# hidasib/GRU4Rec

Measured on NVIDIA H100. Metric: mini-batches/sec, higher is better.
Workload: dtype f32

## Files before the change

### gru4rec_b200/csrc/g4r_fast.cuh

```cuda
#pragma once

constexpr int FK_THREADS = 512;
constexpr int FK_NW = FK_THREADS / 32;
constexpr int FK_G = 48;
constexpr int FK_CT = 32;
constexpr int FK_Q = FK_CT / FK_NW;
constexpr int FK_B = 32;
static_assert(FK_THREADS / 16 == FK_B, "statistics mapping: 16 threads per lane");
constexpr int FK_LDS = 132;


__device__ __forceinline__ void red_release_add(unsigned int* p, unsigned int v) {
  asm volatile("red.release.gpu.global.add.u32 [%0], %1;" :: "l"(p), "r"(v) : "memory");
}
__device__ __forceinline__ unsigned int atom_acqrel_add(unsigned int* p, unsigned int v) {
  unsigned int old;
  asm volatile("atom.acq_rel.gpu.global.add.u32 %0, [%1], %2;" : "=r"(old) : "l"(p), "r"(v) : "memory");
  return old;
}
__device__ __forceinline__ void wait_ge(const unsigned int* p, unsigned int target) {
  while (ld_acquire_u32(p) < target) { }
}
__device__ __forceinline__ uint32_t smem_u32(const void* p) { return (uint32_t)__cvta_generic_to_shared(p); }
__device__ __forceinline__ void mbar_init(uint64_t* bar, unsigned int count) {
// ... 42 lines not shown
  const int tid = threadIdx.x;
  if (s >= n_steps) return;
  const int M = md.wM[s];
  const int* cbeg = md.pCbeg + (size_t)s * (md.NCH + 1);
  const bool hc = chunk < md.NCH;
  const int cb = hc ? cbeg[chunk] : 0, ce = hc ? cbeg[chunk + 1] : 0;
  if (tid < FK_CT) {
    int it = 0, pos = 0;
    if (cb + tid < ce) { it = md.pItem[(size_t)s * md.NP + cb + tid]; pos = md.pPos[(size_t)s * md.NP + cb + tid]; }
    sm.sIt[buf][tid] = it; sm.sPos[buf][tid] = pos;
  }
  if (tid >= 32 && tid < 32 + FK_B) {
    const int b = tid - 32;
    sm.sTc[buf][b] = b < M ? md.pTcol[(size_t)s * md.B + b] : -1;
    sm.sYit[buf][b] = b < M ? md.wY[(size_t)s * md.B + b] : 0;
  }
  if (tid == 64) { sm.sCb[buf][0] = cb; sm.sCb[buf][1] = ce; }
}

template <class SM>
__device__ __forceinline__ void fk_prefetch_rows(const ModelDev& md, SM& sm, int s, int n_steps, int buf, bool pw) {
  if (s >= n_steps) return;
  const int tid = threadIdx.x;
  const int M = md.wM[s];
  const int cb = sm.sCb[buf][0], ce = sm.sCb[buf][1];
  const int nj = ce - cb;
  const bool ada = md.adapt == G4R_ADAPT_ADAGRAD, mom = md.mom > 0.f;
  const unsigned int rowb = (unsigned int)md.ldL * 4u;
  uint64_t* bar = reinterpret_cast<uint64_t*>(&sm.mbar);
  const int ntab = 1 + (ada ? 1 : 0) + (mom ? 1 : 0);
  const int ncopy = nj * ntab + (pw ? M : 0);
  if (tid == 0) {
    const unsigned int total = rowb * (unsigned int)ncopy;
    asm volatile("fence.proxy.async.global;" ::: "memory");
    if (total > 0) mbar_expect_tx(bar, total);
    else asm volatile("mbarrier.arrive.shared::cta.b64 _, [%0];" :: "r"(smem_u32(bar)) : "memory");
  }
  if ((tid & 31) == 0) {
    for (int i = tid >> 5; i < ncopy; i += FK_NW) {
      if (i < nj * ntab) {
        const int j = i / ntab, t = i % ntab;
        const size_t off = (size_t)sm.sIt[buf][j] * md.ldL;
        if (t == 0) tma_row(sm.sS + j * FK_LDS, md.Wy + off, rowb, bar);
        else if (t == 1 && ada) tma_row(sm.sAcc + j * FK_LDS, md.Wy_acc + off, rowb, bar);
        else tma_row(sm.sVel + j * FK_LDS, md.Wy_vel + off, rowb, bar);
      } else {
        const int b = i - nj * ntab;
        tma_row(sm.sTW + b * FK_LDS, md.Wy + (size_t)sm.sYit[buf][b] * md.ldL, rowb, bar);
      }
    }
  }
  if (false) {
  } else if (tid >= 64 && tid < 64 + FK_CT) {
    const int j = tid - 64;
    if (j < nj) {
      const int it = sm.sIt[buf][j];
      float bz = md.By[it];
      sm.sByP[j] = bz;
      if (md.logq > 0.f) bz -= (sm.sPos[buf][j] < M) ? md.logP0t[it] : md.logP0s[it];
      sm.sBias[j] = bz;
      sm.sByA[j] = ada ? md.By_acc[it] : 0.f;
      sm.sByV[j] = mom ? md.By_vel[it] : 0.f;
    }
  } else if (tid >= 96 && tid < 96 + FK_B) {
    const int b = tid - 96;
    if (pw && b < M) {
      const int it = sm.sYit[buf][b];
      float bz = md.By[it];
      if (md.logq > 0.f) bz -= md.logP0t[it];
      sm.sTB[b] = bz;
    }
// ... 556 lines not shown
        if (m == 0) { sc = sm.sD + k0 + j; ss = FK_LDS; } else { sc = (m == 1 ? sm.gDr : sm.gDz) + j; ss = FR_U; }
        o = jm * FK_LDS + q * 4;
      } else {
        vec = sm.sD + q * 4; sc = sm.gHr + k0 + j; ss = FK_LDS;
        o = j * FK_LDS + q * 4;
      }
      float4 g = make_float4(0.f, 0.f, 0.f, 0.f);
#pragma unroll 4
      for (int b = 0; b < M; b++) {
        const float4 a = ld4(vec + b * FK_LDS);
        const float d = sc[b * ss];
        g.x = fmaf(a.x, d, g.x); g.y = fmaf(a.y, d, g.y); g.z = fmaf(a.z, d, g.z); g.w = fmaf(a.w, d, g.w);
      }
      if (k0 + j < L) {
        float* P = colt ? sm.rC[0] : sm.rR[0];
        float* A = colt ? sm.rC[1] : sm.rR[1];
        float* V = colt ? sm.rC[2] : sm.rR[2];
        if (q * 4 + 0 < L) fr_upd(md, ada, mom, g.x, P[o + 0], A[o + 0], V[o + 0]);
        if (q * 4 + 1 < L) fr_upd(md, ada, mom, g.y, P[o + 1], A[o + 1], V[o + 1]);
        if (q * 4 + 2 < L) fr_upd(md, ada, mom, g.z, P[o + 2], A[o + 2], V[o + 2]);
        if (q * 4 + 3 < L) fr_upd(md, ada, mom, g.w, P[o + 3], A[o + 3], V[o + 3]);
      }
    } else {
      const int i = t - ncol - nrow, m = i / FR_U, j = i % FR_U;
      if (k0 + j < L) {
        float g = 0.f;
        for (int b = 0; b < M; b++) g = g + (m == 0 ? sm.sD[b * FK_LDS + k0 + j] : (m == 1 ? sm.gDr : sm.gDz)[b * FR_U + j]);
        fr_upd(md, ada, mom, g, sm.rB[0][i], sm.rB[1][i], sm.rB[2][i]);
      }
    }
  }
}
template <class SM>
__device__ __forceinline__ void fk_stage_y(const ModelDev& md, SM& sm, int M, float* hnext) {
  const LayerDev& ly = md.layer[0];
  const int ldL = ly.ldL, kw = ldL / 4, n1 = FK_B * kw, total = hnext ? 2 * n1 : n1;
  for (int i0 = 0; i0 < total; i0 += 4 * FK_THREADS) {
    float4 v[4];
#pragma unroll
    for (int u = 0; u < 4; u++) {
      const int i = i0 + u * FK_THREADS + (int)threadIdx.x;
      v[u] = make_float4(0.f, 0.f, 0.f, 0.f);
      if (i < n1) { const int rr = i / kw; if (rr < M) v[u] = ld4(ly.y + (size_t)rr * ldL + (i % kw) * 4); }
      else if (i < total) { const int sl = sm.gIdx[(i - n1) / kw]; if (sl >= 0) v[u] = ld4(ly.H + (size_t)sl * ldL + ((i - n1) % kw) * 4); }
    }
#pragma unroll
    for (int u = 0; u < 4; u++) {
      const int i = i0 + u * FK_THREADS + (int)threadIdx.x;
      if (i < n1) st4(sm.sY + (i / kw) * FK_LDS + (i % kw) * 4, v[u]);
      else if (i < total) st4(hnext + ((i - n1) / kw) * FK_LDS + ((i - n1) % kw) * 4, v[u]);
    }
  }
}

#include "g4r_fastc.cuh"

template <bool CL>
__global__ void __launch_bounds__(FK_THREADS, 1) k_fast_t(int slot, int n_steps, FastSync* fs, unsigned long long* tstamp) {
  using SM = typename std::conditional<CL, FastSmemC, FastSmemR>::type;
  extern __shared__ __align__(128) unsigned char fk_raw[];
  SM& sm = *reinterpret_cast<SM*>(fk_raw);
  const ModelDev& md = MD;
  const LayerDev& ly = md.layer[0];
  const int cta = blockIdx.x, ncta = gridDim.x;
  const int tid = threadIdx.x, lane = tid & 31, warp = tid >> 5;
  const int chunk = cta;
  const bool has_chunk = chunk < md.NCH;
  const int G = CL ? (int)cl_size() : md.ldL / 4;
  const bool gru = cta < G;
  const bool pw = loss_pairwise(md.loss);
  const bool ada = md.adapt == G4R_ADAPT_ADAGRAD, mom = md.mom > 0.f;
  const int ldL = md.ldL, B = md.B;
  const int kw = ldL / 4;
  uint64_t* bar = reinterpret_cast<uint64_t*>(&sm.mbar);
  unsigned int bar_epoch = 0, gepoch = 0, stats_target = 0;
  const int in_ctas = min(B, ncta - G);
#ifdef G4R_CF_FINE
#define FK_FTS(s_) ((tstamp && cta == 0 && (s_) < 500 && n_steps >= 1000) ? tstamp + (size_t)((s_) + 500) * 16 : nullptr)
#define FK_STAMP_OK(s_) ((s_) < 500)
#else
#define FK_FTS(s_) ((unsigned long long*)nullptr)
#define FK_STAMP_OK(s_) true
#endif
#define FK_STAMP(k) do { if (tstamp && cta == 0 && tid == 0 && FK_STAMP_OK(s)) { unsigned long long t_; asm volatile("mov.u64 %0, %%globaltimer;" : "=l"(t_)); tstamp[(size_t)s * 16 + (k)] = t_; } } while (0)
  if (tid == 0) { mbar_init(bar, 1); asm volatile("fence.mbarrier_init.release.cluster;" ::: "memory"); }
  fk_load_idx(md, sm, 0, n_steps, chunk, 0);
  __syncthreads();
  fk_prefetch_rows(md, sm, 0, n_steps, 0, pw);
  ClusterCtx cc = {0, 1, 0, 0};
  if constexpr (CL) {
    if (gru) {
      cc = cf_init(md, sm);
      cf_load_resident(md, sm, cc);
      if (n_steps > 0) {
        fk_stage_lanes(md, sm, 0, md.wM[0]);
        cf_f1(md, sm, cc, 0, false, nullptr, 0u, nullptr);
        cf_f2(md, sm, cc, 0, nullptr);
        __syncthreads();
        if (tid == 0) red_release_add(&fs->h_ready, 1u);
      }
    }
  } else {
    if (gru) {
      fr_load_resident(md, sm, 4 * cta);
      if (n_steps > 0) {
        fk_stage_lanes(md, sm, 0, md.wM[0]);
        stage_rows4(sm.gH[0], FK_LDS, FK_B, kw, [&](int rr) -> const float* { const int sl = sm.gIdx[rr]; return sl >= 0 ? ly.H + (size_t)sl * ldL : nullptr; });
        fr_f1(md, sm, 0, 4 * cta, sm.gH[0], nullptr, 0u);
        fk_group_barrier(fs, gepoch, G);
        fr_f2(md, sm, 0, 4 * cta, sm.gH[0]);
        __syncthreads();
        if (tid == 0) red_release_add(&fs->h_ready, 1u);
      }
    }
  }
  for (int s = 0; s < n_steps; s++) {
    const int buf = s & 1;
    const int M = md.wM[s];
    const int sti = md.wSti[s];
    const int N = M + (sti >= 0 ? md.S : 0);
    FK_STAMP(0);
    fk_load_idx(md, sm, s + 1, n_steps, chunk, buf ^ 1);
    const bool gru_next = !CL && gru && s + 1 < n_steps;
    if (gru_next && tid < FK_B) {
      const int M1 = md.wM[s + 1];
      sm.gIdx[tid] = tid < M1 ? md.wSlot[(size_t)(s + 1) * B + tid] : -1;
      sm.gIdx[FK_B + tid] = tid < M1 ? md.wX[(size_t)(s + 1) * B + tid] : 0;
      sm.gIdx[2 * FK_B + tid] = tid < M1 ? md.wF[(size_t)(s + 1) * B + tid] : 0;
    }
    if (tid == 0) wait_ge(&fs->h_ready, (unsigned int)(s + 1) * (unsigned int)G);
    __syncthreads();
    if constexpr (CL) stage_rows4(sm.sY, FK_LDS, FK_B, kw, [&](int rr) -> const float* { return rr < M ? ly.y + (size_t)rr * ldL : nullptr; });
    else fk_stage_y(md, sm, M, gru_next ? sm.gH[(s + 1) & 1] : nullptr);
    mbar_wait(bar, (unsigned int)(s & 1));
    __syncthreads();
    FK_STAMP(1);
    const int cb = sm.sCb[buf][0], ce = sm.sCb[buf][1];
    const int nj = ce - cb;
    if (pw) {
      for (int b = warp; b < FK_B; b += FK_NW) {
        if (b < M) {
          float a = 0.f;
          if (lane < kw) {
            const float4 y = ld4(sm.sY + b * FK_LDS + lane * 4), w = ld4(sm.sTW + b * FK_LDS + lane * 4);
            a = fmaf(w.x, y.x, a); a = fmaf(w.y, y.y, a); a = fmaf(w.z, y.z, a); a = fmaf(w.w, y.w, a);
          }
          a = warp_sum(a);
          if (lane == 0) sm.sT[b] = act_fwd(md.fact, a + sm.sTB[b]);
        }
      }
    }
    {
      float accq[FK_Q];
#pragma unroll
      for (int q = 0; q < FK_Q; q++) accq[q] = 0.f;
      const float* yr = sm.sY + lane * FK_LDS;
      for (int c4 = 0; c4 < kw; c4++) {
        const float4 y = ld4(yr + c4 * 4);
#pragma unroll
        for (int q = 0; q < FK_Q; q++) {
          if (warp + FK_NW * q < nj) {
            const float4 w = ld4(sm.sS + (warp + FK_NW * q) * FK_LDS + c4 * 4);
            accq[q] = fmaf(y.x, w.x, accq[q]); accq[q] = fmaf(y.y, w.y, accq[q]); accq[q] = fmaf(y.z, w.z, accq[q]); accq[q] = fmaf(y.w, w.w, accq[q]);
          }
        }
      }
// ... 88 lines not shown
        const float m = mg;
        float* rs = md.RS + (size_t)b * G4R_NSTAT;
        float loss = 0.f, r0 = m, r1 = Z, r2 = 0.f, r3 = 0.f, r4 = 0.f, r5 = tt;
        if (md.loss == G4R_LOSS_XE) { const float pt = __fdiv_rn(expf(T - m), Z); loss = -logf(pt + G4R_EPS_LOG); r2 = pt; r5 = T; }
        else if (md.loss == G4R_LOSS_XE_LOGIT) { loss = logf(Z) - (T - m); r5 = T; }
        else if (md.loss == G4R_LOSS_BPR_MAX) { r2 = __fdiv_rn(A, Z); r3 = __fdiv_rn(Q, Z); r4 = __fdiv_rn(D, Z); loss = -logf(r2 + G4R_EPS_LOG) + md.bpreg * r3; }
        else if (md.loss == G4R_LOSS_TOP1_MAX) { r2 = __fdiv_rn(A, Z); r4 = __fdiv_rn(D, Z); loss = r2; }
        else if (md.loss == G4R_LOSS_BPR) { loss = A; r4 = D; }
        else { const float c = sigmoidf_(tt * tt); loss = (float)M * (__fdiv_rn(A, (float)N) - __fdiv_rn(c, (float)(M + md.S_cfg))); r4 = D; }
        st4(rs, make_float4(r0, r1, r2, r3));
        st4(rs + 4, make_float4(r4, r5, loss, 0.f));
        red_release_add(&fs->stats, 1u);
      }
    }
    stats_target += (unsigned int)M;
    if (tid == 0) wait_ge(&fs->stats, stats_target);
    __syncthreads();
    FK_STAMP(2);
    if (tid < M * 2) st4(sm.sRS + tid * 4, ld4(md.RS + tid * 4));
    __syncthreads();
    if (chunk == 0 && tid == 0) {
      float c = 0.f;
      for (int b = 0; b < M; b++) c += sm.sRS[b * 8 + 6];
      c = __fdiv_rn(c, (float)md.B);
      md.cost[s] = c;
      if (c != c) atomicExch(md.nanflag, 1);
    }
    FK_STAMP(11);
    for (int i = tid; i < FK_CT * FK_B; i += FK_THREADS) {
      const int jj = i / FK_B, b = i % FK_B;
      sm.sG[i] = (jj < nj && b < M) ? loss_grad_elem(md, sm.sRS + (size_t)b * 8, sm.sO[i], sm.sTc[buf][b] == cb + jj, M, N) : 0.f;
    }
    __syncthreads();
    for (int jj = warp; jj < nj; jj += FK_THREADS / 32) {
      float a = (lane < M) ? sm.sG[jj * FK_B + lane] : 0.f;
      a = warp_sum(a);
      if (lane == 0) sm.sDby[jj] = a;
    }
    FK_STAMP(12);
    float* part = md.part + (size_t)(has_chunk ? chunk : 0) * md.B * ldL;
    if (has_chunk) {
      for (int t = tid; t < nj * kw; t += FK_THREADS) {
        const int jj = t / kw, q4 = t % kw;
        float4 d = make_float4(0.f, 0.f, 0.f, 0.f);
        for (int bb = 0; bb < M; bb++) {
          const float4 y = ld4(sm.sY + bb * FK_LDS + q4 * 4);
          const float g = sm.sG[jj * FK_B + bb];
          d.x = fmaf(g, y.x, d.x); d.y = fmaf(g, y.y, d.y); d.z = fmaf(g, y.z, d.z); d.w = fmaf(g, y.w, d.w);
        }
        st4(sm.sD + jj * FK_LDS + q4 * 4, d);
      }
      for (int t = tid; t < M * kw; t += FK_THREADS) {
        const int bb = t / kw, q4 = t % kw;
        float4 a = make_float4(0.f, 0.f, 0.f, 0.f);
        for (int jj = 0; jj < nj; jj++) {
          const float g = sm.sG[jj * FK_B + bb];
          const float4 w = ld4(sm.sS + jj * FK_LDS + q4 * 4);
          a.x = fmaf(g, w.x, a.x); a.y = fmaf(g, w.y, a.y); a.z = fmaf(g, w.z, a.z); a.w = fmaf(g, w.w, a.w);
        }
        st4(part + (size_t)bb * ldL + q4 * 4, a);
      }
    }
    __syncthreads();
    FK_STAMP(13);
    for (int j = warp; j < nj; j += FK_THREADS / 32) {
      const int item = sm.sIt[buf][j];
      if (j > 0 && sm.sIt[buf][j - 1] == item) continue;
      int je = j + 1;
      while (je < nj && sm.sIt[buf][je] == item) je++;
      if (lane < kw) {
        const float4 p0 = ld4(sm.sS + j * FK_LDS + lane * 4);
        float4 a0 = make_float4(0.f, 0.f, 0.f, 0.f), v0 = a0, al = a0, vl = a0;
        if (ada) a0 = ld4(sm.sAcc + j * FK_LDS + lane * 4);
        if (mom) v0 = ld4(sm.sVel + j * FK_LDS + lane * 4);
        float4 ps = p0;
        for (int k = j; k < je; k++) {
          const float4 g = ld4(sm.sD + k * FK_LDS + lane * 4);
          float4 gs = g;
          if (ada) {
            al.x = a0.x + g.x * g.x; al.y = a0.y + g.y * g.y; al.z = a0.z + g.z * g.z; al.w = a0.w + g.w * g.w;
            gs.x = __fdiv_rn(g.x, sqrtf(al.x + G4R_EPS_ADA)); gs.y = __fdiv_rn(g.y, sqrtf(al.y + G4R_EPS_ADA));
            gs.z = __fdiv_rn(g.z, sqrtf(al.z + G4R_EPS_ADA)); gs.w = __fdiv_rn(g.w, sqrtf(al.w + G4R_EPS_ADA));
          }
          float4 d;
          if (md.lmbd > 0.f) { d.x = md.lr * (gs.x + md.lmbd * p0.x); d.y = md.lr * (gs.y + md.lmbd * p0.y); d.z = md.lr * (gs.z + md.lmbd * p0.z); d.w = md.lr * (gs.w + md.lmbd * p0.w); }
          else { d.x = md.lr * gs.x; d.y = md.lr * gs.y; d.z = md.lr * gs.z; d.w = md.lr * gs.w; }
          if (mom) {
            vl.x = md.mom * v0.x - d.x; vl.y = md.mom * v0.y - d.y; vl.z = md.mom * v0.z - d.z; vl.w = md.mom * v0.w - d.w;
            ps.x += vl.x; ps.y += vl.y; ps.z += vl.z; ps.w += vl.w;
          } else { ps.x -= d.x; ps.y -= d.y; ps.z -= d.z; ps.w -= d.w; }
        }
        const size_t off = (size_t)item * ldL + lane * 4;
        st4(md.Wy + off, ps);
        if (ada) st4(md.Wy_acc + off, al);
        if (mom) st4(md.Wy_vel + off, vl);
      }
      if (lane == 0) {
        const float p0 = sm.sByP[j];
        float a0 = sm.sByA[j], v0 = sm.sByV[j], al = 0.f, vl = 0.f, ps = p0;
        for (int k = j; k < je; k++) {
          const float g = sm.sDby[k];
          float gs = g;
          if (ada) { al = a0 + g * g; gs = __fdiv_rn(g, sqrtf(al + G4R_EPS_ADA)); }
          const float d = md.lmbd > 0.f ? md.lr * (gs + md.lmbd * p0) : md.lr * gs;
          if (mom) { vl = md.mom * v0 - d; ps += vl; } else ps -= d;
        }
        md.By[item] = ps;
        if (ada) md.By_acc[item] = al;
        if (mom) md.By_vel[item] = vl;
      }
    }
    if (has_chunk && nj == 0) for (int i = tid; i < M * ldL; i += FK_THREADS) part[i] = 0.f;
    __syncthreads();
    FK_STAMP(14);
    bar_epoch += 1;
    if (tid == 0) { red_release_add(&fs->bar, 1u); wait_ge(&fs->bar, bar_epoch * (unsigned int)ncta); }
    __syncthreads();
    FK_STAMP(3);
    fk_b1<CL>(md, sm, s, cta, ncta);
    __syncthreads();
    if (tid == 0) red_release_add(&fs->b1_done, 1u);
    FK_STAMP(15);
    fk_prefetch_rows(md, sm, s + 1, n_steps, buf ^ 1, pw);
    FK_STAMP(4);
    if constexpr (CL) {
      if (gru) {
        if (s + 1 < n_steps) fk_stage_lanes(md, sm, s + 1, md.wM[s + 1]);
        cf_backward(md, sm, cc, fs, s, ncta, s + 1 < n_steps, (tstamp && cta == 0 && FK_STAMP_OK(s)) ? tstamp + (size_t)s * 16 : nullptr, FK_FTS(s));
        FK_STAMP(6);
        if (s + 1 < n_steps) {
          cf_f1(md, sm, cc, s + 1, true, &fs->in_done, (unsigned int)(s + 1) * (unsigned int)in_ctas, FK_FTS(s));
          FK_STAMP(7);
          cf_f2(md, sm, cc, s + 1, FK_FTS(s));
          __syncthreads();
          if (tid == 0) red_release_add(&fs->h_ready, 1u);
        } else {
          cl_wait();
        }
        FK_STAMP(8);
      }
    } else if (gru) {
      const int k0 = 4 * cta;
      const float* sHo = sm.gH[s & 1];
      if (tid == 0) wait_ge(&fs->b1_done, (unsigned int)(s + 1) * (unsigned int)ncta);
      __syncthreads();
      fr_b2(md, sm, s, k0, sHo);
      __syncthreads();
      if (tid == 0) red_release_add(&fs->dvec_done, 1u);
      FK_STAMP(5);
      fr_dense(md, sm, s, k0, sHo);
      FK_STAMP(6);
      if (s + 1 < n_steps) {
        fr_f1(md, sm, s + 1, k0, sm.gH[(s + 1) & 1], &fs->in_done, (unsigned int)(s + 1) * (unsigned int)in_ctas);
        fk_group_barrier(fs, gepoch, G);
        FK_STAMP(7);
        fr_f2(md, sm, s + 1, k0, sm.gH[(s + 1) & 1]);
        __syncthreads();
        if (tid == 0) red_release_add(&fs->h_ready, 1u);
      }
      FK_STAMP(8);
    }
    if (!gru && cta < G + in_ctas) {
      const unsigned int* ctr = CL ? &fs->grp : &fs->dvec_done;
      const unsigned int tgt = (unsigned int)(s + 1) * (unsigned int)G;
      if (in_ctas == B && ly.ld3 / 4 <= FK_THREADS) fk_sparse_in_one(md, sm, s, cta - G, ctr, tgt);
      else {
        if (tid == 0) wait_ge(ctr, tgt);
        __syncthreads();
        for (int b = cta - G; b < B; b += in_ctas) { fk_sparse_in(md, sm, s, b); __syncthreads(); }
      }
      __syncthreads();
      if (tid == 0) red_release_add(&fs->in_done, 1u);
    }
  }
  if constexpr (CL) { if (gru) cf_store_resident(md, sm, cc); }
  else { if (gru) fr_store_resident(md, sm, 4 * cta); }
#undef FK_STAMP
}
```

### gru4rec_b200/csrc/g4r_kernels.cuh

```cuda
#pragma once
#include <cuda_runtime.h>
#include <stdint.h>
#include "../../include/g4r.h"

#define G4R_EPS_ADA 1e-6f
#define G4R_EPS_LOG 1e-24f
#define G4R_NSTAT 8

struct ActSpec { int kind; float p1, p2; };
constexpr int MG_CAP = 256;
struct MgDev {
  int R, rank;
  int *gItem, *gPos, *gM, *gX;
  int *mEnt, *mItem, *mCbeg;
  int *mTot;
  int *xEnt, *xItem, *xTot;
  float *DSYall, *DBYall, *INall;
  float* gradFlat; size_t gradCount;
};

struct MgTensor { float *p, *acc, *vel; size_t goff; int count; };
struct TsBuf {
  unsigned char *A1, *A2, *A3, *A4, *A5, *A6, *A7, *A8;
  unsigned char *W1, *W2, *W3, *W4, *B3, *B4, *B5, *B8a, *B8b;
// ... 25 lines not shown
  return t;
}

constexpr int MGS_MAXR = 8;
constexpr int MGS_FLAG_STRIDE = 32;
constexpr int MGS_GRU_CTAS = 48;
enum { MGF_ROWS = 0, MGF_APPLIED = MGS_MAXR, MGF_IN = 2 * MGS_MAXR, MGF_INAPPLIED = 3 * MGS_MAXR, MGF_DENSE = 4 * MGS_MAXR,
       MGF_COUNT = 4 * MGS_MAXR + MGS_MAXR * MGS_GRU_CTAS };
struct ShardDev {
  int R, rank, rows_local, ldW;
  int NA, DSL;
  float* W[MGS_MAXR];
  float* Wx[MGS_MAXR];
  float* inbox[MGS_MAXR];
  float* inboxIn[MGS_MAXR];
  float* denseIn[MGS_MAXR];
  float* mgInLL[MGS_MAXR];
  unsigned int* flags[MGS_MAXR];
  float *W_acc, *W_vel, *Wx_acc, *Wx_vel;
  float* mgIn;
  const int *aEnt, *aItem, *aCbeg;
  const int *xEnt, *xItem, *xTot;
  const int *gX, *gM;
  int* abort;
};
struct FastSync {
  unsigned int bar;      unsigned int p0[31];
  unsigned int stats;    unsigned int p1[31];
  unsigned int h_ready;  unsigned int p2[31];
  unsigned int b1_done;  unsigned int p3[31];
  unsigned int grp;      unsigned int p4[31];
  unsigned int in_done;  unsigned int p5[31];
  unsigned int dvec_done; unsigned int p6[31];
};
struct GridBar { unsigned int count; unsigned int gen; unsigned int pad[30]; };

struct LayerDev {
  int L, ldL, ld2, ld3;
  int in_dim, ld_in;
  float *Wx, *Wx_acc, *Wx_vel;
  float *Wh, *Wh_acc, *Wh_vel;
  float *Wrz, *Wrz_acc, *Wrz_vel;
  float *Bh, *Bh_acc, *Bh_vel;
  float *Wx_g, *Wh_g, *Wrz_g, *Bh_g;
  float *H;
  float *Hold, *r, *z, *ah, *ht, *y;
  float *dvec;
  float *dy;
  float *Hr;
  const float* in;
};

struct ModelDev {
  int n_items, n_layers, B, Bld, S, mode;
  int L, ldL;
  int in0_dim, ld_in0;
  int NP;
  int NCH;
  int loss; ActSpec fact, hact;
  float p_drop_h, p_drop_e, lr, mom, lmbd, bpreg, logq, alpha;
  int adapt; int nn_top1;
  float ap1, ap1c, ap2, ap2c;
  float grad_cap, smoothing;
  const float* gscale;
  float* gnorm2;
  float* stat2;
// ... 1238 lines not shown
```

### gru4rec_b200/csrc/g4r_lib.cu

```cuda
#include <cuda_runtime.h>
#include <algorithm>
#include <cmath>
#include <cstdio>
#include <cstring>
#include <map>
#include <mutex>
#include <string>
#include <vector>
#include "g4r_kernels.cuh"
#include "g4r_misc.cuh"

#define G4R_VERSION 100

static thread_local std::string g_create_error;
struct g4r_handle;
static void eval_release(g4r_handle* h);
static void mg_release(g4r_handle* h);
static void shard_release(g4r_handle* h);
static bool shard_eligible(const g4r_config& c, int n_sm);
static int shard_create(g4r_handle* h);
static bool tc_eligible(const g4r_config& c);
struct TensorInfo;
static int shard_set_tensor(g4r_handle* h, const TensorInfo& t, const float* host);
static int shard_get_tensor(g4r_handle* h, const TensorInfo& t, float* host);
// ... 674 lines not shown
  if (h->two_pass) h->md.export_only = 1;
  if (slot_upload(h->slot, h->md, h->stream) != cudaSuccess) return bail(G4R_ERR_CUDA, "constant upload failed");
  const int B = cfg->batch_size, CAP = h->CAP;
  bool ok = true;
  ok &= cudaMallocHost(&h->hX, (size_t)CAP * B * sizeof(int)) == cudaSuccess;
  ok &= cudaMallocHost(&h->hY, (size_t)CAP * B * sizeof(int)) == cudaSuccess;
  ok &= cudaMallocHost(&h->hSlot, (size_t)CAP * B * sizeof(int)) == cudaSuccess;
  ok &= cudaMallocHost(&h->hF, (size_t)CAP * B) == cudaSuccess;
  ok &= cudaMallocHost(&h->hM, (size_t)CAP * sizeof(int)) == cudaSuccess;
  ok &= cudaMallocHost(&h->hSti, (size_t)CAP * sizeof(int)) == cudaSuccess;
  ok &= cudaMallocHost(&h->hG, (size_t)CAP * sizeof(uint32_t)) == cudaSuccess;
  ok &= cudaMallocHost(&h->hCost, (size_t)CAP * sizeof(float)) == cudaSuccess;
  if (!ok) return bail(G4R_ERR_CUDA, "pinned host allocation failed");
  h->pk_smem = std::max(std::max(score_smem_bytes(h->md.Bld), lossgrad_smem_bytes(h->md.Bld, h->md.ldL)), (size_t)2 * GK * (GB + 1) * sizeof(float));
  if (raise_smem_limit((const void*)k_score, score_smem_bytes(h->md.Bld)) != cudaSuccess ||
      raise_smem_limit((const void*)k_lossgrad, lossgrad_smem_bytes(h->md.Bld, h->md.ldL)) != cudaSuccess ||
      raise_smem_limit((const void*)k_plan, (size_t)h->npow2 * 8 + 1024) != cudaSuccess ||
      raise_smem_limit((const void*)k_persistent, h->pk_smem) != cudaSuccess)
    return bail(G4R_ERR_INVALID, "this shape needs more shared memory per block than the device offers (batch_size / layer width / n_sample too large for the step scratch)");
  {
    int per_sm = 0;
    cudaOccupancyMaxActiveBlocksPerMultiprocessor(&per_sm, k_persistent, PK_THREADS, h->pk_smem);
    int coop = 0; cudaDeviceGetAttribute(&coop, cudaDevAttrCooperativeLaunch, cfg->device);
    h->pk_blocks = (per_sm >= 1 && coop) ? h->n_sm : 0;
  }
  {
    const ModelDev& m = h->md;
    raise_smem_limit((const void*)k_fast_t<false>, sizeof(FastSmemR));
    int per_sm = 0;
    cudaOccupancyMaxActiveBlocksPerMultiprocessor(&per_sm, k_fast_t<false>, FK_THREADS, sizeof(FastSmemR));
    const bool plain_opt = m.adapt <= G4R_ADAPT_ADAGRAD && !h->phase_only;
    h->fast_ok = plain_opt && h->pk_blocks > 0 && per_sm >= 1 && m.mode == 0 && m.n_layers == 1 && m.ldL <= 128 && m.B <= FK_B && h->n_sm >= FK_G + 1 && m.NCH <= 160 &&
                 2 * m.L <= FK_W1 * FK_G && m.L <= FK_W2 * FK_G &&
                 (m.adapt == G4R_ADAPT_ADAGRAD ? m.Wy_acc != nullptr : true);
    h->fastc_ok = plain_opt && cfg->step_mode == 3 && h->fastc_grid >= FC_CLUSTER * 2 && m.mode == 0 && m.n_layers == 1 && m.ldL <= 128 && m.B <= FK_B &&
                  m.NCH <= h->fastc_grid && (m.adapt == G4R_ADAPT_ADAGRAD ? m.Wy_acc != nullptr : true);
    cudaMallocHost(&h->hFlags, 4 * sizeof(int));
  }
  if (h->tc_ok) {
    if (ts_opt_in(h) != G4R_OK) return bail(G4R_ERR_CUDA, "k_ts_gemm: shared memory / cluster opt-in failed");
    h->fast_ok = false; h->fastc_ok = false;
  }
  if (cfg->step_mode == 1 && h->pk_blocks == 0) return bail(G4R_ERR_INVALID, "persistent mode unavailable (cooperative launch / shared memory)");
  if (h->md.shardR > 0) {
    const int src = shard_create(h);
    if (src) return bail(src, h->err);
    h->fast_ok = false; h->fastc_ok = false;
  }
  if (cudaStreamSynchronize(h->stream) != cudaSuccess) return bail(G4R_ERR_CUDA, "init sync failed");
  *out = h;
  return G4R_OK;
}

extern "C" void* g4r_stream(g4r_handle* h) { return h ? (void*)h->stream : nullptr; }
extern "C" int64_t g4r_kernel_launches(const g4r_handle* h) { return h ? h->launches : 0; }

static TensorInfo* find_tensor(g4r_handle* h, const char* name) {
  auto it = h->tensors.find(name ? name : "");
  return it == h->tensors.end() ? nullptr : &it->second;
}
extern "C" int g4r_tensor_shape(g4r_handle* h, const char* name, int64_t* rows, int64_t* cols) {
  if (!h) return G4R_ERR_INVALID;
  TensorInfo* t = find_tensor(h, name);
  if (!t) FAIL(G4R_ERR_INVALID, std::string("unknown tensor ") + (name ? name : "(null)"));
  if (rows) *rows = t->rows;
  if (cols) *cols = t->cols;
// ... 555 lines not shown
```

Before: 28450.

## Offload GRU CTAs' output-row updates to partner CTAs in the non-cluster fast kernel

In the non-cluster persistent kernel, GRU-owning CTAs no longer compute dS·y or apply the output-embedding optimizer updates. They write their loss gradients to global memory, and a dedicated partner CTA fetches them and performs the row updates. That lets the GRU CTAs move straight on to the barrier and the recurrent backward/forward work on the critical path. A new rows_done counter orders the next step's TMA row prefetch after all row updates finish, and next-step H staging moves into the GRU branch. The change needs extra CTAs (a new eligibility check), adds a global round-trip of gradients and extra syncs, and moves the async-proxy fence onto each issuing warp.

```diff
diff --git a/gru4rec_b200/csrc/g4r_fast.cuh b/gru4rec_b200/csrc/g4r_fast.cuh
--- a/gru4rec_b200/csrc/g4r_fast.cuh
+++ b/gru4rec_b200/csrc/g4r_fast.cuh
@@ -98,11 +98,11 @@
   const int ncopy = nj * ntab + (pw ? M : 0);
   if (tid == 0) {
     const unsigned int total = rowb * (unsigned int)ncopy;
-    asm volatile("fence.proxy.async.global;" ::: "memory");
     if (total > 0) mbar_expect_tx(bar, total);
     else asm volatile("mbarrier.arrive.shared::cta.b64 _, [%0];" :: "r"(smem_u32(bar)) : "memory");
   }
   if ((tid & 31) == 0) {
+    asm volatile("fence.proxy.async.global;" ::: "memory");
     for (int i = tid >> 5; i < ncopy; i += FK_NW) {
       if (i < nj * ntab) {
         const int j = i / ntab, t = i % ntab;
@@ -725,25 +725,130 @@
   }
 }
 template <class SM>
-__device__ __forceinline__ void fk_stage_y(const ModelDev& md, SM& sm, int M, float* hnext) {
-  const LayerDev& ly = md.layer[0];
-  const int ldL = ly.ldL, kw = ldL / 4, n1 = FK_B * kw, total = hnext ? 2 * n1 : n1;
-  for (int i0 = 0; i0 < total; i0 += 4 * FK_THREADS) {
-    float4 v[4];
-#pragma unroll
-    for (int u = 0; u < 4; u++) {
-      const int i = i0 + u * FK_THREADS + (int)threadIdx.x;
-      v[u] = make_float4(0.f, 0.f, 0.f, 0.f);
-      if (i < n1) { const int rr = i / kw; if (rr < M) v[u] = ld4(ly.y + (size_t)rr * ldL + (i % kw) * 4); }
-      else if (i < total) { const int sl = sm.gIdx[(i - n1) / kw]; if (sl >= 0) v[u] = ld4(ly.H + (size_t)sl * ldL + ((i - n1) % kw) * 4); }
-    }
-#pragma unroll
-    for (int u = 0; u < 4; u++) {
-      const int i = i0 + u * FK_THREADS + (int)threadIdx.x;
-      if (i < n1) st4(sm.sY + (i / kw) * FK_LDS + (i % kw) * 4, v[u]);
-      else if (i < total) st4(hnext + ((i - n1) / kw) * FK_LDS + ((i - n1) % kw) * 4, v[u]);
-    }
-  }
+__device__ __forceinline__ void fk_part(SM& sm, float* part, int M, int nj, int ldL) {
+  const int kw = ldL / 4;
+  for (int t = threadIdx.x; t < M * kw; t += FK_THREADS) {
+    const int bb = t / kw, q4 = t % kw;
+    float4 a = make_float4(0.f, 0.f, 0.f, 0.f);
+    for (int jj = 0; jj < nj; jj++) {
+      const float g = sm.sG[jj * FK_B + bb];
+      const float4 w = ld4(sm.sS + jj * FK_LDS + q4 * 4);
+      a.x = fmaf(g, w.x, a.x); a.y = fmaf(g, w.y, a.y); a.z = fmaf(g, w.z, a.z); a.w = fmaf(g, w.w, a.w);
+    }
+    st4(part + (size_t)bb * ldL + q4 * 4, a);
+  }
+}
+template <class SM>
+__device__ __forceinline__ void fk_dsy(SM& sm, int M, int nj, int kw) {
+  for (int t = threadIdx.x; t < nj * kw; t += FK_THREADS) {
+    const int jj = t / kw, q4 = t % kw;
+    float4 d = make_float4(0.f, 0.f, 0.f, 0.f);
+    for (int bb = 0; bb < M; bb++) {
+      const float4 y = ld4(sm.sY + bb * FK_LDS + q4 * 4);
+      const float g = sm.sG[jj * FK_B + bb];
+      d.x = fmaf(g, y.x, d.x); d.y = fmaf(g, y.y, d.y); d.z = fmaf(g, y.z, d.z); d.w = fmaf(g, y.w, d.w);
+    }
+    st4(sm.sD + jj * FK_LDS + q4 * 4, d);
+  }
+}
+template <class SM>
+__device__ __forceinline__ void fk_update_rows(const ModelDev& md, SM& sm, int buf, int nj, int kw) {
+  const int lane = threadIdx.x & 31, warp = threadIdx.x >> 5, ldL = md.ldL;
+  const bool ada = md.adapt == G4R_ADAPT_ADAGRAD, mom = md.mom > 0.f;
+  for (int j = warp; j < nj; j += FK_NW) {
+    const int item = sm.sIt[buf][j];
+    if (j > 0 && sm.sIt[buf][j - 1] == item) continue;
+    int je = j + 1;
+    while (je < nj && sm.sIt[buf][je] == item) je++;
+    if (lane < kw) {
+      const float4 p0 = ld4(sm.sS + j * FK_LDS + lane * 4);
+      float4 a0 = make_float4(0.f, 0.f, 0.f, 0.f), v0 = a0, al = a0, vl = a0;
+      if (ada) a0 = ld4(sm.sAcc + j * FK_LDS + lane * 4);
+      if (mom) v0 = ld4(sm.sVel + j * FK_LDS + lane * 4);
+      float4 ps = p0;
+      for (int k = j; k < je; k++) {
+        const float4 g = ld4(sm.sD + k * FK_LDS + lane * 4);
+        float4 gs = g;
+        if (ada) {
+          al.x = a0.x + g.x * g.x; al.y = a0.y + g.y * g.y; al.z = a0.z + g.z * g.z; al.w = a0.w + g.w * g.w;
+          gs.x = __fdiv_rn(g.x, sqrtf(al.x + G4R_EPS_ADA)); gs.y = __fdiv_rn(g.y, sqrtf(al.y + G4R_EPS_ADA));
+          gs.z = __fdiv_rn(g.z, sqrtf(al.z + G4R_EPS_ADA)); gs.w = __fdiv_rn(g.w, sqrtf(al.w + G4R_EPS_ADA));
+        }
+        float4 d;
+        if (md.lmbd > 0.f) { d.x = md.lr * (gs.x + md.lmbd * p0.x); d.y = md.lr * (gs.y + md.lmbd * p0.y); d.z = md.lr * (gs.z + md.lmbd * p0.z); d.w = md.lr * (gs.w + md.lmbd * p0.w); }
+        else { d.x = md.lr * gs.x; d.y = md.lr * gs.y; d.z = md.lr * gs.z; d.w = md.lr * gs.w; }
+        if (mom) {
+          vl.x = md.mom * v0.x - d.x; vl.y = md.mom * v0.y - d.y; vl.z = md.mom * v0.z - d.z; vl.w = md.mom * v0.w - d.w;
+          ps.x += vl.x; ps.y += vl.y; ps.z += vl.z; ps.w += vl.w;
+        } else { ps.x -= d.x; ps.y -= d.y; ps.z -= d.z; ps.w -= d.w; }
+      }
+      const size_t off = (size_t)item * ldL + lane * 4;
+      st4(md.Wy + off, ps);
+      if (ada) st4(md.Wy_acc + off, al);
+      if (mom) st4(md.Wy_vel + off, vl);
+    }
+    if (lane == 0) {
+      const float p0 = sm.sByP[j];
+      float a0 = sm.sByA[j], v0 = sm.sByV[j], al = 0.f, vl = 0.f, ps = p0;
+      for (int k = j; k < je; k++) {
+        const float g = sm.sDby[k];
+        float gs = g;
+        if (ada) { al = a0 + g * g; gs = __fdiv_rn(g, sqrtf(al + G4R_EPS_ADA)); }
+        const float d = md.lmbd > 0.f ? md.lr * (gs + md.lmbd * p0) : md.lr * gs;
+        if (mom) { vl = md.mom * v0 - d; ps += vl; } else ps -= d;
+      }
+      md.By[item] = ps;
+      if (ada) md.By_acc[item] = al;
+      if (mom) md.By_vel[item] = vl;
+    }
+  }
+}
+template <class SM>
+__device__ __forceinline__ void fk_dby(SM& sm, int M, int nj) {
+  const int lane = threadIdx.x & 31, warp = threadIdx.x >> 5;
+  for (int jj = warp; jj < nj; jj += FK_NW) {
+    float a = (lane < M) ? sm.sG[jj * FK_B + lane] : 0.f;
+    a = warp_sum(a);
+    if (lane == 0) sm.sDby[jj] = a;
+  }
+}
+struct FkPartner { int nj, it; float g[2]; };
+__device__ __forceinline__ FkPartner fk_partner_fetch(const ModelDev& md, int s, int g, int M) {
+  const int tid = threadIdx.x;
+  const int* cbeg = md.pCbeg + (size_t)s * (md.NCH + 1);
+  const int cb = g < md.NCH ? cbeg[g] : 0;
+  FkPartner r;
+  r.nj = g < md.NCH ? cbeg[g + 1] - cb : 0;
+  r.it = (tid < r.nj) ? md.pItem[(size_t)s * md.NP + cb + tid] : 0;
+#pragma unroll
+  for (int u = 0; u < 2; u++) {
+    const int i = u * FK_THREADS + tid, jj = i / FK_B, b = i % FK_B;
+    r.g[u] = (jj < r.nj && b < M) ? md.O[(size_t)(cb + jj) * md.Bld + b] : 0.f;
+  }
+  return r;
+}
+template <class SM>
+__device__ int fk_partner_stage(const ModelDev& md, SM& sm, const FkPartner& r, int buf, int M, int kw) {
+  static_assert(FK_CT * FK_B == 2 * FK_THREADS, "fk_partner_fetch: two dL/do entries per thread");
+  const int tid = threadIdx.x, lane = tid & 31, warp = tid >> 5, nj = r.nj;
+  const bool ada = md.adapt == G4R_ADAPT_ADAGRAD, mom = md.mom > 0.f;
+  __syncthreads();
+  if (tid < FK_CT) sm.sIt[buf][tid] = r.it;
+  sm.sG[tid] = r.g[0]; sm.sG[FK_THREADS + tid] = r.g[1];
+  __syncthreads();
+  for (int j = warp; j < nj; j += FK_NW) {
+    const int it = sm.sIt[buf][j];
+    const size_t off = (size_t)it * md.ldL + lane * 4;
+    if (lane < kw) {
+      st4(sm.sS + j * FK_LDS + lane * 4, ld4(md.Wy + off));
+      if (ada) st4(sm.sAcc + j * FK_LDS + lane * 4, ld4(md.Wy_acc + off));
+      if (mom) st4(sm.sVel + j * FK_LDS + lane * 4, ld4(md.Wy_vel + off));
+    }
+    if (lane == 0) { sm.sByP[j] = md.By[it]; sm.sByA[j] = ada ? md.By_acc[it] : 0.f; sm.sByV[j] = mom ? md.By_vel[it] : 0.f; }
+  }
+  asm volatile("fence.proxy.async.shared::cta;" ::: "memory");
+  fk_dby(sm, M, nj);
+  return nj;
 }
 
 #include "g4r_fastc.cuh"
@@ -762,12 +867,12 @@
   const int G = CL ? (int)cl_size() : md.ldL / 4;
   const bool gru = cta < G;
   const bool pw = loss_pairwise(md.loss);
-  const bool ada = md.adapt == G4R_ADAPT_ADAGRAD, mom = md.mom > 0.f;
   const int ldL = md.ldL, B = md.B;
   const int kw = ldL / 4;
   uint64_t* bar = reinterpret_cast<uint64_t*>(&sm.mbar);
   unsigned int bar_epoch = 0, gepoch = 0, stats_target = 0;
   const int in_ctas = min(B, ncta - G);
+  const int partner_of = (!CL && cta >= G + in_ctas && cta < 2 * G + in_ctas) ? cta - G - in_ctas : -1;
 #ifdef G4R_CF_FINE
 #define FK_FTS(s_) ((tstamp && cta == 0 && (s_) < 500 && n_steps >= 1000) ? tstamp + (size_t)((s_) + 500) * 16 : nullptr)
 #define FK_STAMP_OK(s_) ((s_) < 500)
@@ -823,8 +928,7 @@
     }
     if (tid == 0) wait_ge(&fs->h_ready, (unsigned int)(s + 1) * (unsigned int)G);
     __syncthreads();
-    if constexpr (CL) stage_rows4(sm.sY, FK_LDS, FK_B, kw, [&](int rr) -> const float* { return rr < M ? ly.y + (size_t)rr * ldL : nullptr; });
-    else fk_stage_y(md, sm, M, gru_next ? sm.gH[(s + 1) & 1] : nullptr);
+    stage_rows4(sm.sY, FK_LDS, FK_B, kw, [&](int rr) -> const float* { return rr < M ? ly.y + (size_t)rr * ldL : nullptr; });
     mbar_wait(bar, (unsigned int)(s & 1));
     __syncthreads();
     FK_STAMP(1);
@@ -979,98 +1083,34 @@
       sm.sG[i] = (jj < nj && b < M) ? loss_grad_elem(md, sm.sRS + (size_t)b * 8, sm.sO[i], sm.sTc[buf][b] == cb + jj, M, N) : 0.f;
     }
     __syncthreads();
-    for (int jj = warp; jj < nj; jj += FK_THREADS / 32) {
-      float a = (lane < M) ? sm.sG[jj * FK_B + lane] : 0.f;
-      a = warp_sum(a);
-      if (lane == 0) sm.sDby[jj] = a;
+    if (!CL && gru) {
+      for (int i = tid; i < nj * FK_B; i += FK_THREADS) {
+        const int jj = i / FK_B, b = i % FK_B;
+        if (b < M) md.O[(size_t)(cb + jj) * md.Bld + b] = sm.sG[i];
+      }
+    } else {
+      fk_dby(sm, M, nj);
     }
     FK_STAMP(12);
     float* part = md.part + (size_t)(has_chunk ? chunk : 0) * md.B * ldL;
-    if (has_chunk) {
-      for (int t = tid; t < nj * kw; t += FK_THREADS) {
-        const int jj = t / kw, q4 = t % kw;
-        float4 d = make_float4(0.f, 0.f, 0.f, 0.f);
-        for (int bb = 0; bb < M; bb++) {
-          const float4 y = ld4(sm.sY + bb * FK_LDS + q4 * 4);
-          const float g = sm.sG[jj * FK_B + bb];
-          d.x = fmaf(g, y.x, d.x); d.y = fmaf(g, y.y, d.y); d.z = fmaf(g, y.z, d.z); d.w = fmaf(g, y.w, d.w);
-        }
-        st4(sm.sD + jj * FK_LDS + q4 * 4, d);
-      }
-      for (int t = tid; t < M * kw; t += FK_THREADS) {
-        const int bb = t / kw, q4 = t % kw;
-        float4 a = make_float4(0.f, 0.f, 0.f, 0.f);
-        for (int jj = 0; jj < nj; jj++) {
-          const float g = sm.sG[jj * FK_B + bb];
-          const float4 w = ld4(sm.sS + jj * FK_LDS + q4 * 4);
-          a.x = fmaf(g, w.x, a.x); a.y = fmaf(g, w.y, a.y); a.z = fmaf(g, w.z, a.z); a.w = fmaf(g, w.w, a.w);
-        }
-        st4(part + (size_t)bb * ldL + q4 * 4, a);
-      }
-    }
-    __syncthreads();
-    FK_STAMP(13);
-    for (int j = warp; j < nj; j += FK_THREADS / 32) {
-      const int item = sm.sIt[buf][j];
-      if (j > 0 && sm.sIt[buf][j - 1] == item) continue;
-      int je = j + 1;
-      while (je < nj && sm.sIt[buf][je] == item) je++;
-      if (lane < kw) {
-        const float4 p0 = ld4(sm.sS + j * FK_LDS + lane * 4);
-        float4 a0 = make_float4(0.f, 0.f, 0.f, 0.f), v0 = a0, al = a0, vl = a0;
-        if (ada) a0 = ld4(sm.sAcc + j * FK_LDS + lane * 4);
-        if (mom) v0 = ld4(sm.sVel + j * FK_LDS + lane * 4);
-        float4 ps = p0;
-        for (int k = j; k < je; k++) {
-          const float4 g = ld4(sm.sD + k * FK_LDS + lane * 4);
-          float4 gs = g;
-          if (ada) {
-            al.x = a0.x + g.x * g.x; al.y = a0.y + g.y * g.y; al.z = a0.z + g.z * g.z; al.w = a0.w + g.w * g.w;
-            gs.x = __fdiv_rn(g.x, sqrtf(al.x + G4R_EPS_ADA)); gs.y = __fdiv_rn(g.y, sqrtf(al.y + G4R_EPS_ADA));
-            gs.z = __fdiv_rn(g.z, sqrtf(al.z + G4R_EPS_ADA)); gs.w = __fdiv_rn(g.w, sqrtf(al.w + G4R_EPS_ADA));
-          }
-          float4 d;
-          if (md.lmbd > 0.f) { d.x = md.lr * (gs.x + md.lmbd * p0.x); d.y = md.lr * (gs.y + md.lmbd * p0.y); d.z = md.lr * (gs.z + md.lmbd * p0.z); d.w = md.lr * (gs.w + md.lmbd * p0.w); }
-          else { d.x = md.lr * gs.x; d.y = md.lr * gs.y; d.z = md.lr * gs.z; d.w = md.lr * gs.w; }
-          if (mom) {
-            vl.x = md.mom * v0.x - d.x; vl.y = md.mom * v0.y - d.y; vl.z = md.mom * v0.z - d.z; vl.w = md.mom * v0.w - d.w;
-            ps.x += vl.x; ps.y += vl.y; ps.z += vl.z; ps.w += vl.w;
-          } else { ps.x -= d.x; ps.y -= d.y; ps.z -= d.z; ps.w -= d.w; }
-        }
-        const size_t off = (size_t)item * ldL + lane * 4;
-        st4(md.Wy + off, ps);
-        if (ada) st4(md.Wy_acc + off, al);
-        if (mom) st4(md.Wy_vel + off, vl);
-      }
-      if (lane == 0) {
-        const float p0 = sm.sByP[j];
-        float a0 = sm.sByA[j], v0 = sm.sByV[j], al = 0.f, vl = 0.f, ps = p0;
-        for (int k = j; k < je; k++) {
-          const float g = sm.sDby[k];
-          float gs = g;
-          if (ada) { al = a0 + g * g; gs = __fdiv_rn(g, sqrtf(al + G4R_EPS_ADA)); }
-          const float d = md.lmbd > 0.f ? md.lr * (gs + md.lmbd * p0) : md.lr * gs;
-          if (mom) { vl = md.mom * v0 - d; ps += vl; } else ps -= d;
-        }
-        md.By[item] = ps;
-        if (ada) md.By_acc[item] = al;
-        if (mom) md.By_vel[item] = vl;
-      }
-    }
-    if (has_chunk && nj == 0) for (int i = tid; i < M * ldL; i += FK_THREADS) part[i] = 0.f;
-    __syncthreads();
-    FK_STAMP(14);
-    bar_epoch += 1;
-    if (tid == 0) { red_release_add(&fs->bar, 1u); wait_ge(&fs->bar, bar_epoch * (unsigned int)ncta); }
-    __syncthreads();
-    FK_STAMP(3);
-    fk_b1<CL>(md, sm, s, cta, ncta);
-    __syncthreads();
-    if (tid == 0) red_release_add(&fs->b1_done, 1u);
-    FK_STAMP(15);
-    fk_prefetch_rows(md, sm, s + 1, n_steps, buf ^ 1, pw);
-    FK_STAMP(4);
     if constexpr (CL) {
+      if (has_chunk) { fk_dsy(sm, M, nj, kw); fk_part(sm, part, M, nj, ldL); }
+      __syncthreads();
+      FK_STAMP(13);
+      fk_update_rows(md, sm, buf, nj, kw);
+      if (has_chunk && nj == 0) for (int i = tid; i < M * ldL; i += FK_THREADS) part[i] = 0.f;
+      __syncthreads();
+      FK_STAMP(14);
+      bar_epoch += 1;
+      if (tid == 0) { red_release_add(&fs->bar, 1u); wait_ge(&fs->bar, bar_epoch * (unsigned int)ncta); }
+      __syncthreads();
+      FK_STAMP(3);
+      fk_b1<CL>(md, sm, s, cta, ncta);
+      __syncthreads();
+      if (tid == 0) red_release_add(&fs->b1_done, 1u);
+      FK_STAMP(15);
+      fk_prefetch_rows(md, sm, s + 1, n_steps, buf ^ 1, pw);
+      FK_STAMP(4);
       if (gru) {
         if (s + 1 < n_steps) fk_stage_lanes(md, sm, s + 1, md.wM[s + 1]);
         cf_backward(md, sm, cc, fs, s, ncta, s + 1 < n_steps, (tstamp && cta == 0 && FK_STAMP_OK(s)) ? tstamp + (size_t)s * 16 : nullptr, FK_FTS(s));
@@ -1086,38 +1126,87 @@
         }
         FK_STAMP(8);
       }
-    } else if (gru) {
-      const int k0 = 4 * cta;
-      const float* sHo = sm.gH[s & 1];
-      if (tid == 0) wait_ge(&fs->b1_done, (unsigned int)(s + 1) * (unsigned int)ncta);
+      if (!gru && cta < G + in_ctas) {
+        const unsigned int tgt = (unsigned int)(s + 1) * (unsigned int)G;
+        if (in_ctas == B && ly.ld3 / 4 <= FK_THREADS) fk_sparse_in_one(md, sm, s, cta - G, &fs->grp, tgt);
+        else {
+          if (tid == 0) wait_ge(&fs->grp, tgt);
+          __syncthreads();
+          for (int b = cta - G; b < B; b += in_ctas) { fk_sparse_in(md, sm, s, b); __syncthreads(); }
+        }
+        __syncthreads();
+        if (tid == 0) red_release_add(&fs->in_done, 1u);
+      }
+    } else {
+      if (has_chunk) fk_part(sm, part, M, nj, ldL);
+      if (has_chunk && nj == 0) for (int i = tid; i < M * ldL; i += FK_THREADS) part[i] = 0.f;
       __syncthreads();
-      fr_b2(md, sm, s, k0, sHo);
+      FK_STAMP(13);
+      bar_epoch += 1;
+      if (tid == 0) { red_release_add(&fs->bar, 1u); wait_ge(&fs->bar, bar_epoch * (unsigned int)ncta); }
       __syncthreads();
-      if (tid == 0) red_release_add(&fs->dvec_done, 1u);
-      FK_STAMP(5);
-      fr_dense(md, sm, s, k0, sHo);
-      FK_STAMP(6);
-      if (s + 1 < n_steps) {
-        fr_f1(md, sm, s + 1, k0, sm.gH[(s + 1) & 1], &fs->in_done, (unsigned int)(s + 1) * (unsigned int)in_ctas);
-        fk_group_barrier(fs, gepoch, G);
-        FK_STAMP(7);
-        fr_f2(md, sm, s + 1, k0, sm.gH[(s + 1) & 1]);
+      FK_STAMP(3);
+      fk_b1<CL>(md, sm, s, cta, ncta);
+      __syncthreads();
+      if (tid == 0) red_release_add(&fs->b1_done, 1u);
+      FK_STAMP(15);
+      const bool nxt = s + 1 < n_steps;
+      const unsigned int rows_target = (unsigned int)(s + 1) * (unsigned int)ncta;
+      if (gru) {
+        const int k0 = 4 * cta;
+        const float* sHo = sm.gH[s & 1];
+        float* hnext = sm.gH[(s + 1) & 1];
+        if (nxt) stage_rows4(hnext, FK_LDS, FK_B, kw, [&](int rr) -> const float* { const int sl = sm.gIdx[rr]; return sl >= 0 ? ly.H + (size_t)sl * ldL : nullptr; });
         __syncthreads();
-        if (tid == 0) red_release_add(&fs->h_ready, 1u);
-      }
-      FK_STAMP(8);
-    }
-    if (!gru && cta < G + in_ctas) {
-      const unsigned int* ctr = CL ? &fs->grp : &fs->dvec_done;
-      const unsigned int tgt = (unsigned int)(s + 1) * (unsigned int)G;
-      if (in_ctas == B && ly.ld3 / 4 <= FK_THREADS) fk_sparse_in_one(md, sm, s, cta - G, ctr, tgt);
-      else {
-        if (tid == 0) wait_ge(ctr, tgt);
+        FK_STAMP(14);
+        if (tid == 0) { red_release_add(&fs->rows_done, 1u); wait_ge(&fs->b1_done, (unsigned int)(s + 1) * (unsigned int)ncta); }
         __syncthreads();
-        for (int b = cta - G; b < B; b += in_ctas) { fk_sparse_in(md, sm, s, b); __syncthreads(); }
-      }
-      __syncthreads();
-      if (tid == 0) red_release_add(&fs->in_done, 1u);
+        FK_STAMP(4);
+        fr_b2(md, sm, s, k0, sHo);
+        __syncthreads();
+        if (tid == 0) red_release_add(&fs->dvec_done, 1u);
+        FK_STAMP(5);
+        fr_dense(md, sm, s, k0, sHo);
+        FK_STAMP(6);
+        if (nxt) {
+          fr_f1(md, sm, s + 1, k0, hnext, &fs->in_done, (unsigned int)(s + 1) * (unsigned int)in_ctas);
+          fk_group_barrier(fs, gepoch, G);
+          FK_STAMP(7);
+          fr_f2(md, sm, s + 1, k0, hnext);
+          __syncthreads();
+          if (tid == 0) red_release_add(&fs->h_ready, 1u);
+          if (tid == 0) wait_ge(&fs->rows_done, rows_target);
+          __syncthreads();
+          fk_prefetch_rows(md, sm, s + 1, n_steps, buf ^ 1, pw);
+        }
+        FK_STAMP(8);
+      } else {
+        const FkPartner pc = partner_of >= 0 ? fk_partner_fetch(md, s, partner_of, M) : FkPartner{0, 0, {0.f, 0.f}};
+        for (int pass = 0, njp = nj; pass < (partner_of >= 0 ? 2 : 1); pass++) {
+          if (pass == 1) njp = fk_partner_stage(md, sm, pc, buf, M, kw);
+          fk_dsy(sm, M, njp, kw);
+          __syncthreads();
+          fk_update_rows(md, sm, buf, njp, kw);
+        }
+        __syncthreads();
+        if (tid == 0) red_release_add(&fs->rows_done, 1u);
+        if (cta < G + in_ctas) {
+          const unsigned int tgt = (unsigned int)(s + 1) * (unsigned int)G;
+          if (in_ctas == B && ly.ld3 / 4 <= FK_THREADS) fk_sparse_in_one(md, sm, s, cta - G, &fs->dvec_done, tgt);
+          else {
+            if (tid == 0) wait_ge(&fs->dvec_done, tgt);
+            __syncthreads();
+            for (int b = cta - G; b < B; b += in_ctas) { fk_sparse_in(md, sm, s, b); __syncthreads(); }
+          }
+          __syncthreads();
+          if (tid == 0) red_release_add(&fs->in_done, 1u);
+        }
+        if (nxt) {
+          if (tid == 0) wait_ge(&fs->rows_done, rows_target);
+          __syncthreads();
+          fk_prefetch_rows(md, sm, s + 1, n_steps, buf ^ 1, pw);
+        }
+      }
     }
   }
   if constexpr (CL) { if (gru) cf_store_resident(md, sm, cc); }
diff --git a/gru4rec_b200/csrc/g4r_kernels.cuh b/gru4rec_b200/csrc/g4r_kernels.cuh
--- a/gru4rec_b200/csrc/g4r_kernels.cuh
+++ b/gru4rec_b200/csrc/g4r_kernels.cuh
@@ -81,6 +81,7 @@
   unsigned int grp;      unsigned int p4[31];
   unsigned int in_done;  unsigned int p5[31];
   unsigned int dvec_done; unsigned int p6[31];
+  unsigned int rows_done; unsigned int p7[31];
 };
 struct GridBar { unsigned int count; unsigned int gen; unsigned int pad[30]; };
 
diff --git a/gru4rec_b200/csrc/g4r_lib.cu b/gru4rec_b200/csrc/g4r_lib.cu
--- a/gru4rec_b200/csrc/g4r_lib.cu
+++ b/gru4rec_b200/csrc/g4r_lib.cu
@@ -730,6 +730,7 @@
     const bool plain_opt = m.adapt <= G4R_ADAPT_ADAGRAD && !h->phase_only;
     h->fast_ok = plain_opt && h->pk_blocks > 0 && per_sm >= 1 && m.mode == 0 && m.n_layers == 1 && m.ldL <= 128 && m.B <= FK_B && h->n_sm >= FK_G + 1 && m.NCH <= 160 &&
                  2 * m.L <= FK_W1 * FK_G && m.L <= FK_W2 * FK_G &&
+                 h->pk_blocks >= 2 * (m.ldL / 4) + std::min(m.B, h->pk_blocks - m.ldL / 4) &&
                  (m.adapt == G4R_ADAPT_ADAGRAD ? m.Wy_acc != nullptr : true);
     h->fastc_ok = plain_opt && cfg->step_mode == 3 && h->fastc_grid >= FC_CLUSTER * 2 && m.mode == 0 && m.n_layers == 1 && m.ldL <= 128 && m.B <= FK_B &&
                   m.NCH <= h->fastc_grid && (m.adapt == G4R_ADAPT_ADAGRAD ? m.Wy_acc != nullptr : true);
```

Result: faster. 29830, median of 6 (+4.9%).
